# pytorch/audio

Measured on AMD Instinct MI355X. Metric: audio-sec/sec MelSpectrogram (b=256, 16kHz, n_fft=400, n_mels=80), higher is better.
Workload: dtype f32; 1 GPU; MelSpectrogram n_fft=400 hop=160 n_mels=80, batch=256 x 10 s @16 kHz fp32 per GPU (BASELINE configs[1]); per_gpu_batch=256

## Files before the change

### audio_amd/_lib.py

```python
from __future__ import annotations

import ctypes as C
import os
import threading

_HERE = os.path.dirname(os.path.abspath(__file__))
LIB_PATH = os.path.join(_HERE, "lib", "libaudio_amd.so")
if os.environ.get("AAMD_USE_LAB_LIB"):
    LIB_PATH = os.path.join(_HERE, "lib", "libaudio_amd_lab.so")

AAMD_OK = 0
PAD_MODES = {"reflect": 0, "constant": 1, "replicate": 2, "circular": 3}


class StftDesc(C.Structure):
    _fields_ = [
        ("rows", C.c_int64), ("length", C.c_int64), ("row_stride", C.c_int64),
        ("n_fft", C.c_int32), ("hop", C.c_int32), ("pad", C.c_int32), ("center", C.c_int32),
        ("pad_mode", C.c_int32), ("onesided", C.c_int32), ("n_frames", C.c_int32),
        ("scale", C.c_float), ("power", C.c_float),
    ]


class MelBands(C.Structure):
    _fields_ = [
        ("n_mels", C.c_int32), ("max_width", C.c_int32),
        ("lo", C.c_void_p), ("width", C.c_void_p), ("weights", C.c_void_p), ("lane_order", C.c_void_p),
        ("table400", C.c_void_p), ("table_sig", C.c_int32),
    ]


class MfccFused(C.Structure):
    _fields_ = [("dct_frag", C.c_void_p), ("n_mfcc", C.c_int32), ("pass_", C.c_int32), ("multiplier", C.c_float),
                ("amin", C.c_float), ("db_multiplier", C.c_float), ("top_db", C.c_float), ("group_max", C.c_void_p),
                ("rows_per_group", C.c_int64), ("tile_min", C.c_void_p), ("fix_count", C.c_void_p),
                ("tile_list", C.c_void_p)]


class ResampleBands(C.Structure):
    _fields_ = [("n_tiles", C.c_int32), ("tap_span", C.c_int32), ("tap_lo", C.POINTER(C.c_int32))]


_lib = None
# ... 10 lines not shown
class KaldiDesc(C.Structure):
    _fields_ = [("n_samples", C.c_int64), ("n_frames", C.c_int64), ("n_fft", C.c_int32), ("shift", C.c_int32),
                ("win", C.c_int32), ("snip_edges", C.c_int32), ("preemphasis", C.c_float),
                ("remove_dc_offset", C.c_int32), ("raw_energy", C.c_int32), ("energy_floor", C.c_float),
                ("use_power", C.c_int32), ("use_log", C.c_int32), ("energy_col", C.c_int32), ("first_col", C.c_int32),
                ("n_cols", C.c_int32), ("dither", C.c_float), ("noise", C.c_void_p), ("n_utt", C.c_int64),
                ("utt_stride", C.c_int64)]


_SIGS = {
    "aamd_abi_version": (C.c_int, []),
    "aamd_last_error": (C.c_char_p, []),
    "aamd_set_kernel_policy": (C.c_int, [C.c_int]),
    "aamd_mel400_table_dwords": (C.c_int64, [C.c_int32, C.c_int32]),
    "aamd_mel400_table_build": (C.c_int, [C.POINTER(MelBands), _P, _P]),
    "aamd_device_info": (C.c_int, [C.c_char_p, C.c_int32, C.POINTER(C.c_int32), C.POINTER(C.c_int64)]),
    "aamd_box_probe": (C.c_int, [_P, C.c_int32, C.c_int32, _P]),
    "aamd_spectrogram_f32": (C.c_int, [_P, _P, _P, _P, C.POINTER(StftDesc), _P]),
    "aamd_melspectrogram_f32": (C.c_int, [_P, _P, _P, C.POINTER(MelBands), _P, C.POINTER(StftDesc), _P]),
    "aamd_melspectrogram_db_f32": (C.c_int, [_P, _P, _P, C.POINTER(MelBands), _P, C.POINTER(StftDesc), C.c_float,
                                             C.c_float, C.c_float, _P, C.c_int64, _P]),
    "aamd_melspectrogram_lognorm_f32": (C.c_int, [_P, _P, _P, C.POINTER(MelBands), _P, C.POINTER(StftDesc), C.c_float,
                                                  _P, _P, C.c_int64, _P]),
    "aamd_melspectrogram_pcm16_f32": (C.c_int, [_P, _P, _P, C.POINTER(MelBands), _P, C.POINTER(StftDesc), C.c_float,
                                                _P, _P, C.c_int64, _P]),
    "aamd_melspectrogram_pcm16_interleaved_f32": (C.c_int, [_P, C.c_int32, _P, _P, C.POINTER(MelBands), _P,
                                                            C.POINTER(StftDesc), C.c_float, _P, _P, C.c_int64, _P]),
    "aamd_melspectrogram_lowp_f32": (C.c_int, [_P, C.c_int32, _P, _P, C.POINTER(MelBands), _P, C.POINTER(StftDesc), _P]),
    "aamd_spectrogram_grad_f32": (C.c_int, [_P, _P, _P, C.c_int64, C.c_float, _P]),
    "aamd_melspectrogram_grad_f32": (C.c_int, [_P, _P, C.POINTER(MelBands), C.c_int64, C.c_int32, C.c_int32, C.c_float, _P]),
# ... 114 lines not shown
```

### audio_amd/csrc/c_api.hip

```cpp
#include <hip/hip_runtime.h>

#include <atomic>
#include <cmath>
#include <cstdlib>
#include <cstdio>
#include <cstring>
#include <map>
#include <mutex>
#include <utility>
#include <string>

#include "../../include/audio_amd.h"
#include "db_mfcc.h"
#include "f64_paths.h"
#include "feat_post.h"
#include "fftconv.h"
#include "fftconv_os.h"
#include "fftconv_fdr.h"
#include "istft.h"
#include "kaldi_generic.h"
#include "vocoder.h"
#include "stft_pow2.h"
#include "istft400.h"
#include "lfilter.h"
// ... 133 lines not shown
  g.pad_mode = d->pad_mode; g.onesided = d->onesided; g.n_frames = d->n_frames;
  g.n_freq = d->onesided ? d->n_fft / 2 + 1 : d->n_fft;
  g.scale = d->scale; g.power = d->power;
  g.n_stages = plan_radices(d->n_fft, g.radix);
  if (g.n_stages < 0) return fail(AAMD_EUNSUPPORTED, "audio_amd: n_fft has too many prime factors");
  return AAMD_OK;
}

int validate_bands(const aamd_mel_bands* b, int n_freq, MelBandsDev& mb) {
  AAMD_CHECK_ARG(b != nullptr, "null mel bands");
  AAMD_CHECK_ARG(b->n_mels >= 1 && b->max_width >= 1 && b->max_width <= n_freq, "bad mel band table");
  AAMD_CHECK_ARG(b->lo && b->width && b->weights, "null mel band pointers");
  mb.n_mels = b->n_mels; mb.max_width = b->max_width;
  mb.lo = b->lo; mb.width = b->width; mb.weights = b->weights; mb.order = b->lane_order;
  mb.table400 = b->table400;
  mb.table_sig = b->table400 ? b->table_sig : 0;
  return AAMD_OK;
}

template <int EPI, int E>
int launch_pow2(const StftGeom& g, const MelBandsDev& mb, const float* wav, const float* window,
                const float* twiddle, float* out, hipStream_t s) {
  const int64_t pairs_per_row = (g.n_frames + 1) / 2;
  const int64_t n_pairs = g.rows * pairs_per_row;
  if (n_pairs == 0) return AAMD_OK;
  size_t lds = (size_t)p2::kWaves * p2::Cfg<E>::lds_complex * sizeof(p2::C32);
  if (EPI == EPI_MEL && p2::mel_in_lds(mb.n_mels, mb.max_width))
    lds += (size_t)p2::mel_lds_floats(mb.n_mels, mb.max_width) * sizeof(float);
  auto kern = p2::stft_pow2_kernel<E, EPI>;
  if (lds > 48 * 1024)
    AAMD_HIP(hipFuncSetAttribute(reinterpret_cast<const void*>(kern),
// ... 209 lines not shown
  if (n_mels < 1 || max_width < 1) return 0;
  if (m400::mel_ws(max_width) > m400::kMelMaxTaps + 4 || m400::mel_rounds(n_mels) > m400::kMelMaxRounds) return 0;
  return m400::mel_tab_dwords(n_mels, max_width);
}

int aamd_mel400_table_build(const aamd_mel_bands* bands, float* table_out, void* stream) {
  DeviceScope dev_scope_(table_out);
  MelBandsDev mb{};
  int rc = validate_bands(bands, 201, mb);
  if (rc != AAMD_OK) return rc;
  AAMD_CHECK_ARG(table_out != nullptr, "null table buffer");
  if (aamd_mel400_table_dwords(mb.n_mels, mb.max_width) == 0)
    return fail(AAMD_EUNSUPPORTED, "audio_amd: filterbank outside the radix-20x20 kernel (n_mels > 160 or band > 62 bins)");
  mb.table400 = nullptr;
  hipLaunchKernelGGL(m400::mel_tab_build_kernel, dim3(1), dim3(256), 0, (hipStream_t)stream, mb, table_out);
  return launch_check();
}

int aamd_device_info(char* name, int32_t name_len, int32_t* cu_count, int64_t* hbm_bytes) {
  int dev = 0;
  AAMD_HIP(hipGetDevice(&dev));
  hipDeviceProp_t dp;
  AAMD_HIP(hipGetDeviceProperties(&dp, dev));
  if (name && name_len > 0) {
    std::snprintf(name, (size_t)name_len, "%s", dp.gcnArchName);
  }
  if (cu_count) *cu_count = dp.multiProcessorCount;
  if (hbm_bytes) *hbm_bytes = (int64_t)dp.totalGlobalMem;
  return AAMD_OK;
}
// ... 1455 lines not shown
```

### audio_amd/csrc/melspec400.h

```cpp
#pragma once
#include <type_traits>
#include "hd.h"
#include "stft_generic.h"
#include "resample_mfma.h"

namespace aamd {
namespace m400 {

constexpr int kN = 400;
constexpr int kPad = 200;
constexpr int kFramesPerWave = 6;
#ifndef AAMD_M400_WAVES
#define AAMD_M400_WAVES 12
#define AAMD_M400_MINWAVES 3
#endif
constexpr int kWavesPerBlock = AAMD_M400_WAVES;
constexpr int kTOff[20] = {0, 260, 520, 652, 784, 916, 1444, 1576, 128, 388,
                           2104, 2232, 2364, 1708, 1840, 1048, 1180, 1312, 1972, 2492};
constexpr int kTBufDwords = 2492 + 128;
constexpr int kTRow = 44;
constexpr int kTPair = 20 * kTRow;
constexpr int kLdsDwordsPerWave = 3 * kTPair;
constexpr int kPK = 208;
constexpr int kPPair = 416;
// ... 636 lines not shown

template <int NR>
AAMD_HD void mel_regs_load(const LaneConst& c, const MelTab& mt, MelRegs<NR>& h) {
#pragma unroll
  for (int r = 0; r < NR; ++r) {
    const bool on = r < mt.n_rounds;
    const int row = r * kMelSlots + c.pi;
#if defined(__HIP_DEVICE_COMPILE__)
    h.nc[r] = on ? __builtin_amdgcn_readfirstlane(mt.rc[r]) : 0;
#else
    h.nc[r] = on ? mt.rc[r] : 0;
#endif
    const int poff = on ? 2 * mt.lo2[row] : 0;
    const int mel = on ? mt.row_mel[row] : -1;
    h.pm[r] = (int)(((unsigned)mel << 16) | (unsigned)poff);
  }
}

AAMD_HD constexpr int sig_chunks(int sig, int r) { return (sig >> (4 * r)) & 15; }
constexpr int kSigHtk80 = 0x4221, kSigSlaney80 = 0x4211;

template <int NR = kMelMaxRounds, int SIG = 0, bool FENCED = false>
AAMD_HD void phase_c(const LaneConst& c, const MelTab& mt, const float* lds,
                     float (&acc_a)[NR], float (&acc_b)[NR], const MelRegs<NR>* h = nullptr) {
  const float* Pp = lds + kPPair * c.p;
  const float* wt0 = mt.w + c.pi * mt.ws;
#pragma unroll
  for (int r = 0; r < NR; ++r) {
    float sa = 0.0f, sb = 0.0f;
#if defined(__HIP_DEVICE_COMPILE__)
// ... 164 lines not shown
    const float v = mfcc_frag_value(dct, n_mels, n_mfcc, t, s, lane, j);
    const uint16_t hi = rsm::f16_bits(v);
    const uint16_t lo = rsm::f16_bits(v - rsm::f16_value(hi));
    fh[mfcc_frag_piece(t, s, 0, lane) * 8 + j] = hi;
    fh[mfcc_frag_piece(t, s, 1, lane) * 8 + j] = lo;
  }
}

__global__ void __launch_bounds__(256) mel_tab_build_kernel(MelBandsDev mb, float* __restrict__ out) {
  MelTab mt{};
  mel_tab_rounds(threadIdx.x, blockDim.x, mb, out, mt);
  __syncthreads();
  mel_tab_fill(threadIdx.x, blockDim.x, mb, out, mt);
}

template <int LAB, int EPI, int H = 8, typename TIn = float, int NR = kMelMaxRounds, int SIG = 0>
__global__ void __launch_bounds__(64 * kWavesPerBlock, AAMD_M400_MINWAVES)
melspec400_kernel(const TIn* __restrict__ wav, const float* __restrict__ window,
                  const float* __restrict__ tw400, MelBandsDev mb, float* __restrict__ out,
                  int64_t rows, int64_t length, int64_t row_stride, int n_frames, float scale,
                  int tiles_per_row, int64_t n_tiles, int tiles_per_block, int in_aligned,
                  int out_wide, Epi400 epi) {
  extern __shared__ __attribute__((aligned(16))) float smem400[];
  unsigned fix_base = 0, fix_cnt = 0;
#if defined(AAMD_LAB) && defined(AAMD_MFCC_FIXUP_RETURNS)
  if (EPI == EPI400_MFCC && epi.fixup != 0) return;
#endif
  if (EPI == EPI400_MFCC && epi.fixup != 0) {
    int* const cnt = reinterpret_cast<int*>(smem400);
    if (threadIdx.x == 0) *cnt = 0;
// ... 38 lines not shown
#endif
  long long lab_t0 = 0;
  if (LAB & 1024) lab_t0 = wall_clock64();
  if ((LAB & 1048576) && lane == 0) {
    long long* rec = reinterpret_cast<long long*>(epi.fix_count);
    const int w = blockIdx.x * kWavesPerBlock + wave;
    rec[4 * w] = (long long)clock64();
    rec[4 * w + 1] = wall_clock64();
  }
  using HC = Hop<H>;
  constexpr int kHop = HC::hop;
  float* lds = smem400 + wave * HC::lds_dwords;
  const unsigned s_addr = (unsigned)(uintptr_t)(lds + kSOff);

  float* const_tab = smem400 + kWavesPerBlock * HC::lds_dwords;
  const_tab_build(threadIdx.x, blockDim.x, window, tw400, scale, const_tab);
  MelTab mt{};
  const int tab_dwords = (EPI != EPI400_SPEC) ? mel_tab_dwords(mb.n_mels, mb.max_width) : 0;
  int* queue = reinterpret_cast<int*>(const_tab + kConstDwords + tab_dwords);
  constexpr bool kIoWave = (LAB & 16777216) != 0;
  constexpr int kNio = kIoWave ? ((LAB & 67108864) ? 2 : 1) : 0;
  if (threadIdx.x == 0) *queue = kWavesPerBlock - kNio;
  float* frag_lds = const_tab + kConstDwords + tab_dwords + 4;
  constexpr bool kFragLds = (H != 10);
  if (EPI == EPI400_MFCC && (epi.frag_in_lds != 0) != kFragLds) __builtin_trap();
  if (EPI == EPI400_MFCC && kFragLds)
    for (int i = threadIdx.x; i < kMfccFragFloats; i += blockDim.x) frag_lds[i] = epi.dct_frag[i];
  if (EPI != EPI400_SPEC && mb.table400 != nullptr) {
    float* dst = const_tab + kConstDwords;
    for (int i = threadIdx.x; i < tab_dwords; i += blockDim.x) dst[i] = mb.table400[i];
    mel_tab_layout(mb, dst, mt);
    __syncthreads();
  } else {
    if (EPI != EPI400_SPEC) mel_tab_rounds(threadIdx.x, blockDim.x, mb, const_tab + kConstDwords, mt);
    __syncthreads();
    if (EPI != EPI400_SPEC) mel_tab_fill(threadIdx.x, blockDim.x, mb, const_tab + kConstDwords, mt);
    __syncthreads();
  }

  long long lab_t1 = 0;
  if (LAB & 1024) lab_t1 = wall_clock64();
  LaneConst c;
  lane_init(lane, const_tab, c);
  constexpr bool kWinRegs = (EPI != EPI400_MFCC || H != 10) && (((LAB & 8192) != 0) || !(LAB & 262144));
  float winr[20], twr[40];
  if (kWinRegs) {
#pragma unroll
    for (int q = 0; q < 20; ++q) winr[q] = c.win[q];
  }
#ifndef AAMD_M400_TWREG
#define AAMD_M400_TWREG 3
#endif
#ifndef AAMD_M400_TWREG_DB
#define AAMD_M400_TWREG_DB 1
#endif
#ifndef AAMD_M400_TWREG_MFCC
#define AAMD_M400_TWREG_MFCC 2
#endif
  constexpr bool kPlain = H == 8 && std::is_same<TIn, float>::value && LAB == 0;
  constexpr int kTwRegBatches = (LAB & 16384) ? 4
                                : (SIG != 0 && EPI == EPI400_MEL) ? AAMD_M400_TWREG
                                : !kPlain ? 0
                                : EPI == EPI400_SPEC ? 2
                                : (EPI == EPI400_MEL && SIG == 0) ? (NR <= 4 ? 1 : 3)
                                : (EPI == EPI400_MFCC && NR <= 4) ? AAMD_M400_TWREG_MFCC
                                : (EPI == EPI400_MEL_DB && NR <= 4) ? AAMD_M400_TWREG_DB : 0;
  if (kTwRegBatches > 0) {
#pragma unroll
    for (int q = 0; q < 10 * kTwRegBatches; ++q) twr[q] = c.tw[q];
  }
  constexpr bool kHoist = NR <= 4;
  MelRegs<NR> mregs;
  const MelRegs<NR>* mh = nullptr;
  if (EPI != EPI400_SPEC && kHoist) {
    mel_regs_load<NR>(c, mt, mregs);
    mh = &mregs;
  }
  if (SIG != 0) {
    static_assert(SIG == 0 || NR == 4, "filterbank signatures are 4 rounds of 20 mels");
    const int sig_rt = mregs.nc[0] | (mregs.nc[1 % NR] << 4) | (mregs.nc[2 % NR] << 8) | (mregs.nc[3 % NR] << 12);
    if (mt.n_rounds != NR || mt.n_mels != kMelSlots * NR || sig_rt != SIG) __builtin_trap();
  }
  if (EPI == EPI400_MFCC && (mt.n_rounds != NR || mt.n_mels != kMelSlots * NR)) __builtin_trap();
  float nrm_mean[NR], nrm_inv[NR];
  if (EPI == EPI400_MEL_NORM) {
#pragma unroll
    for (int r = 0; r < NR; ++r) {
      const int m = r < mt.n_rounds ? mt.row_mel[r * kMelSlots + c.pi] : -1;
      nrm_mean[r] = m >= 0 ? epi.mean[m] : 0.0f;
      nrm_inv[r] = m >= 0 ? epi.invstd[m] : 0.0f;
    }
  }
  const unsigned long long self_mask = __ballot((c.col == 0) || (c.col == 10));
  using SG = Stage<H, TIn>;
  static_assert(SG::ok, "no staging layout for this hop / input type");
  int spiece[SG::ndma];
#pragma unroll
  for (int k = 0; k < SG::ndma; ++k) spiece[k] = SG::spp * stage_src_piece<H, TIn>(64 * k + lane);

  const int nb = gridDim.x;
  int lb = blockIdx.x;
  if ((nb & 7) == 0) lb = (blockIdx.x & 7) * (nb >> 3) + (blockIdx.x >> 3);
  unsigned blk_first = (unsigned)lb * (unsigned)tiles_per_block;
  unsigned blk_count = 0;
  if (blk_first < (unsigned)n_tiles) {
    blk_count = (unsigned)n_tiles - blk_first;
// ... 155 lines not shown
    for (int i = 0; i < k; ++i) __builtin_amdgcn_s_sleep(17);
  }
  float Xn[HC::nx];
  auto gload = [&](const TileInfo& ti) {
    const TIn* src = wav + (ti.row / InTraits<TIn>::chans) * row_stride + (ti.t0 * kHop - kPad) + (HC::pair_stride * c.p + c.pi);
#pragma unroll
    for (int q = 0; q < HC::nx; ++q) Xn[q] = InTraits<TIn>::get(src + 20 * q, (int)(ti.row % InTraits<TIn>::chans));
  };
  if (LAB & 32768) {
#pragma unroll
    for (int q = 0; q < HC::nx; ++q) Xn[q] = 0.0f;
    if (cur.staged) gload(cur);
  } else if (cur.staged && !(LAB & 8) && !fix) {
    stage_issue(cur);
  }

  long long ph_acc[6] = {0, 0, 0, 0, 0, 0}, ph_t = 0;
  int ph_tiles = 0;
#define AAMD_M400_STAMP(K)                                  \
  if (LAB & 8388608) {                                      \
    const long long now_ = (long long)clock64();            \
    ph_acc[K] += now_ - ph_t;                               \
    ph_t = now_;                                            \
  }
  using mfcc_f32x4 = __attribute__((ext_vector_type(4))) float;
  mfcc_f32x4 cf[kMfccMT];
  const int mfcc_elab = (LAB & 524288) ? epi.lab : 0;
  auto mfcc_finish = [&](int64_t row, int64_t t0) {
#pragma unroll
    for (int t = 0; t < kMfccMT; ++t)
// ... 318 lines not shown
```

### audio_amd/csrc/stft_generic.h

```cpp
#pragma once
#include "hd.h"

namespace aamd {

constexpr int kMaxStages = 16;

struct StftGeom {
  int64_t rows, length, row_stride;
  int n_fft, hop, pad, center, pad_mode, onesided, n_frames, n_freq;
  float scale, power;
  int n_stages;
  int radix[kMaxStages];
};

struct MelBandsDev {
  int n_mels, max_width;
  const int32_t* lo;
  const int32_t* width;
  const float* weights;
  const int32_t* order;
  const float* table400;
  int table_sig;
};

constexpr int kGenThreads = 256;
AAMD_HD int gen_pairs_per_block(int n_fft) {
  int p = 1024 / n_fft;
  return p < 1 ? 1 : (p > 8 ? 8 : p);
}
AAMD_HD int gen_pad(int i) { return i + (i >> 5); }
AAMD_HD int gen_seq_len(int n_fft) { return gen_pad(n_fft - 1) + 1; }
AAMD_HD size_t gen_lds_floats(int n_fft, int n_freq, int pb) {
  return (size_t)2 * n_fft + (size_t)4 * pb * gen_seq_len(n_fft) + (size_t)2 * pb * n_freq;
}
AAMD_HD size_t gen_lds_floats_long(int n_fft, int pb) { return (size_t)4 * pb * gen_seq_len(n_fft); }

template <typename T>
// ... 270 lines not shown
```

### audio_amd/csrc/torch_shim.cpp

```cpp
#include <audio_amd.h>

#include <torch/csrc/inductor/aoti_torch/c/shim.h>
#include <torch/csrc/stable/accelerator.h>
#include <torch/csrc/stable/library.h>
#include <torch/csrc/stable/ops.h>
#include <torch/csrc/stable/tensor.h>
#include <torch/headeronly/core/ScalarType.h>

#include <cmath>
#include <cstdint>
#include <memory>
#include <optional>
#include <string>
#include <type_traits>
#include <vector>

namespace {

using torch::headeronly::ScalarType;
using torch::stable::Tensor;

void check(int rc) {
  STD_TORCH_CHECK(rc == AAMD_OK, aamd_last_error());
}
// ... 60 lines not shown
    b.n_mels = (int32_t)lo.numel();
    b.max_width = (int32_t)weights.size(1);
    b.lo = static_cast<const int32_t*>(lo.data_ptr());
    b.width = static_cast<const int32_t*>(width.data_ptr());
    b.weights = fp(weights);
    b.lane_order = nullptr;
    if (lane_order.has_value()) {
      want_i32(*lane_order, "lane_order");
      same_device(wav, *lane_order);
      b.lane_order = static_cast<const int32_t*>(lane_order->data_ptr());
    }
    b.table400 = nullptr;
    if (table400.has_value()) {
      want_f32(*table400, "table400", 1);
      same_device(wav, *table400);
      STD_TORCH_CHECK(table400->numel() == aamd_mel400_table_dwords(b.n_mels, b.max_width),
                      "audio_amd: table400 does not belong to this band table");
      b.table400 = fp(*table400);
    }
    b.table_sig = b.table400 ? (int32_t)table_sig : 0;
  }
};

Tensor spectrogram(Tensor wav, Tensor window, Tensor twiddle, int64_t n_fft, int64_t hop, int64_t pad, bool center,
                   int64_t pad_mode, bool onesided, int64_t n_frames, double scale, double power) {
  aamd_stft_desc d = make_desc(wav, n_fft, hop, pad, center, pad_mode, onesided, n_frames, scale, power);
  want_f32(window, "window", 1);
  want_f32(twiddle, "twiddle");
  same_device(wav, window);
  same_device(wav, twiddle);
  STD_TORCH_CHECK(window.numel() == n_fft && twiddle.numel() == 2 * n_fft, "audio_amd: window / twiddle size");
  const torch::stable::accelerator::DeviceGuard guard(wav.get_device_index());
  const int64_t n_freq = onesided ? n_fft / 2 + 1 : n_fft;
  Tensor out = torch::stable::new_empty(wav, {d.rows, n_frames, n_freq * (power > 0.0 ? 1 : 2)});
  if (out.numel()) check(aamd_spectrogram_f32(fp(wav), fp(window), fp(twiddle), fpm(out), &d, current_stream(wav)));
// ... 817 lines not shown
```

### audio_amd/functional.py

```python
from __future__ import annotations

import collections
import ctypes as C
import math
import os
import threading
import warnings
import weakref
from typing import List, Optional, Tuple, Union

import numpy as np
import torch
from torch import Tensor

from . import _host
from . import _lib
from . import _shim
from . import _diff
from ._host import create_dct, melscale_fbanks

__all__ = [
    "spectrogram", "inverse_spectrogram", "griffinlim", "phase_vocoder", "pitch_shift", "speed", "amplitude_to_DB", "melscale_fbanks", "create_dct", "resample",
    "lfilter", "biquad", "fftconvolve", "mel_scale", "filtfilt",
    "lowpass_biquad", "highpass_biquad", "allpass_biquad", "bandpass_biquad",
# ... 185 lines not shown
        self.table_sig = 0
        if self.n_freq == 201 and self.lo.is_cuda:
            L = _lib.lib()
            n = L.aamd_mel400_table_dwords(self.n_mels, max_width)
            if n > 0:
                if image is not None and image.shape[0] == n:
                    self.table400 = torch.from_numpy(image).to(device)
                    self.table_sig = _host.mel400_table_signature(image, int(self.n_mels), int(max_width))
                    self.struct.table_sig = self.table_sig
                else:
                    self.table400 = torch.zeros(n, dtype=torch.float32, device=device)
                    with torch.cuda.device(device):
                        _lib.check(L.aamd_mel400_table_build(C.byref(self.struct), self.table400.data_ptr(),
                                                             _lib.current_stream(device)))
                self.struct.table400 = self.table400.data_ptr()


def _mel_bands(fb: Tensor, device) -> MelBandsOnDevice:
    return _tensor_cached(fb, ("bands", str(device)),
                          lambda: MelBandsOnDevice(fb if fb.dtype == torch.float32 else fb.detach().float(), device))


def _get_spec_norms(normalized: Union[str, bool]):
    frame_length_norm, window_norm = False, False
    if isinstance(normalized, str):
        if normalized not in ["frame_length", "window"]:
            raise ValueError("Invalid normalized parameter: {}".format(normalized))
        if normalized == "frame_length":
            frame_length_norm = True
        elif normalized == "window":
# ... 480 lines not shown
                    win_length: int, power: float, normalized, center: bool, pad_mode: str,
                    bands: Optional[MelBandsOnDevice] = None, db=None) -> Tensor:
    _require_device(waveform, "waveform")
    if power is None:
        raise ValueError("audio_amd: MelSpectrogram needs a real power (got None)")
    window = window.to(device=waveform.device, dtype=torch.float32)
    x2 = _rows2d(waveform)
    desc = _stft_desc(x2, pad, window, n_fft, hop_length, power, normalized, center, pad_mode, True)
    if bands is None:
        bands = _mel_bands(fb, waveform.device)
    if bands.n_freq != n_fft // 2 + 1:
        raise RuntimeError(
            f"mat1 and mat2 shapes cannot be multiplied ({desc.n_frames}x{n_fft // 2 + 1} and "
            f"{bands.n_freq}x{bands.n_mels})")
    ops = _ops()
    if ops is not None:
        targs = (x2, _padded_window(window, n_fft), _twiddles(n_fft, waveform.device), bands.lo, bands.width,
                 bands.weights, bands.lane_order, bands.table400, n_fft, hop_length, pad, bool(center), desc.pad_mode, desc.n_frames,
                 desc.scale, desc.power)
        sig = int(bands.table_sig)
        if db is None:
            return ops.mel_spectrogram(*targs, sig)
        multiplier, amin, db_multiplier, group_max, rows_per_group = db
        return ops.mel_spectrogram_db(*targs, multiplier, amin, db_multiplier, group_max, rows_per_group, sig)
    out = torch.empty((desc.rows, desc.n_frames, bands.n_mels), dtype=torch.float32, device=waveform.device)
    if out.numel():
        L = _lib.lib()
        args = (x2.data_ptr(), _padded_window(window, n_fft).data_ptr(), _twiddles(n_fft, waveform.device).data_ptr(),
                C.byref(bands.struct), out.data_ptr(), C.byref(desc))
        if db is None:
            _lib.check(L.aamd_melspectrogram_f32(*args, _lib.current_stream(waveform.device)))
        else:
            multiplier, amin, db_multiplier, group_max, rows_per_group = db
            _lib.check(L.aamd_melspectrogram_db_f32(
                *args, multiplier, amin, db_multiplier, None if group_max is None else group_max.data_ptr(),
                rows_per_group, _lib.current_stream(waveform.device)))
    return out


def _melspectrogram_lowp(waveform: Tensor, pad: int, window: Tensor, fb: Tensor, n_fft: int, hop_length: int,
                         win_length: int, power: float, normalized, center: bool, pad_mode: str) -> Optional[Tensor]:
    if n_fft != 400 or hop_length not in (160, 200) or power != 2.0 or not waveform.is_cuda:
        return None
    dev = waveform.device
# ... 20 lines not shown
def _melspectrogram_plan(waveform: Tensor, pad: int, window: Tensor, fb: Tensor, n_fft: int, hop_length: int,
                         win_length: int, power: float, normalized, center: bool, pad_mode: str):
    ops = _ops()
    if ops is None or power is None:
        return None
    _require_device(waveform, "waveform")
    window_in = window
    window = window.to(device=waveform.device, dtype=torch.float32)
    x2 = _rows2d(waveform)
    if x2.data_ptr() != waveform.data_ptr():
        return None
    desc = _stft_desc(x2, pad, window, n_fft, hop_length, power, normalized, center, pad_mode, True)
    bands = _mel_bands(fb, waveform.device)
    if bands.n_freq != n_fft // 2 + 1:
        return None
    args = (_padded_window(window, n_fft), _twiddles(n_fft, waveform.device), bands.lo, bands.width, bands.weights,
            bands.lane_order, bands.table400, n_fft, hop_length, pad, bool(center), desc.pad_mode, desc.n_frames,
            desc.scale, desc.power, int(bands.table_sig))
    return ops.mel_spectrogram, (x2.shape[0], x2.shape[1]), args, (bands, window, window_in, fb)


def _mel_lognorm(waveform: Tensor, window: Tensor, fb: Tensor, n_fft: int, hop_length: int, gain: float,
                 mean: Tensor, invstddev: Tensor, right_padding: int,
                 bands: Optional[MelBandsOnDevice] = None, interleaved_channels: int = 0) -> Tensor:
    L0 = _lib.lib()
    if interleaved_channels:
        C_ = int(interleaved_channels)
        if waveform.dtype != torch.int16 or waveform.shape[-1] != C_:
            raise ValueError("audio_amd: interleaved PCM must be int16 with a trailing channel dimension")
        n_time = waveform.shape[-2]
        direct = (C_ in (1, 2) and waveform.is_cuda and n_fft == 400 and hop_length in (160, 200) and n_time > 400
                  and not (L0.aamd_set_kernel_policy(-1) & _lib.POLICY_FORCE_GENERIC))
# ... 36 lines not shown
        raise RuntimeError(f"audio_amd: global statistics must have n_mels = {bands.n_mels} entries")
    if pcm16 and not interleaved_channels and not (bands.n_mels <= 160 and bands.max_width <= 62):
        return _mel_lognorm(waveform.to(torch.float32) * (1.0 / 32768.0), window, fb, n_fft, hop_length, gain, mean,
                            invstddev, right_padding, bands)
    T = desc.n_frames
    n_time = x2.shape[-2] if interleaved_channels else x2.shape[1]
    fused_pad = (right_padding > 0 and n_fft == 400 and hop_length in (100, 160, 200) and n_time > 400
                 and bands.n_mels <= 160 and bands.max_width <= 62
                 and not (L0.aamd_set_kernel_policy(-1) & _lib.POLICY_FORCE_GENERIC))
    if interleaved_channels:
        def entry(wav, *rest):
            return L0.aamd_melspectrogram_pcm16_interleaved_f32(wav, int(interleaved_channels), *rest)
    else:
        entry = L0.aamd_melspectrogram_pcm16_f32 if pcm16 else L0.aamd_melspectrogram_lognorm_f32

    def launch(frames: int) -> Tensor:
        out = torch.empty((desc.rows, frames, bands.n_mels), dtype=torch.float32, device=dev)
        if out.numel():
            if frames > T:
                out[:, T:].zero_()
            if T:
                _lib.check(entry(
                    x2.data_ptr(), _padded_window(window, n_fft).data_ptr(), _twiddles(n_fft, dev).data_ptr(),
                    C.byref(bands.struct), out.data_ptr(), C.byref(desc), float(gain), mean.data_ptr(),
                    invstddev.data_ptr(), frames, _lib.current_stream(dev)))
        return out

    if fused_pad:
        try:
            return launch(T + right_padding)
        except RuntimeError as e:
            if "padded feature rows" not in str(e):
                raise
    out = launch(T)
    if right_padding:
        out = torch.nn.functional.pad(out, (0, 0, 0, right_padding))
    return out


# ... 87 lines not shown
            frag = torch.empty((L.aamd_mfcc_frag_floats(),), dtype=torch.float32, device=dev)
            _lib.check(L.aamd_mfcc_frag_build(dct.data_ptr(), bands.n_mels, n_mfcc, frag.data_ptr(), stream))
            state.frag, state.frag_key, state.frag_src = frag, key, weakref.ref(dct)
        n_tiles = int(L.aamd_mfcc_fused_tiles(C.byref(desc)))
        out = torch.empty((desc.rows, desc.n_frames, n_mfcc), dtype=torch.float32, device=dev)
        gmax = _neg_inf.take(n_groups, dev)
        if out.numel() == 0:
            if group_max_hook is not None:
                group_max_hook(gmax)
            return out
        tile_min = torch.empty((n_tiles,), dtype=torch.float32, device=dev)
        count = torch.empty((1,), dtype=torch.int32, device=dev)
        tile_list = torch.empty((n_tiles,), dtype=torch.int32, device=dev)
        f = _lib.MfccFused(state.frag.data_ptr(), n_mfcc, 0, float(db[0]), float(db[1]), float(db[2]), float(top_db),
                           gmax.data_ptr(), max(packed, 1), tile_min.data_ptr(), count.data_ptr(), tile_list.data_ptr())
        args = (x2.data_ptr(), _padded_window(window, n_fft).data_ptr(), _twiddles(n_fft, dev).data_ptr(),
                C.byref(bands.struct), out.data_ptr(), C.byref(desc))
        _lib.check(L.aamd_mfcc_fused_f32(*args, C.byref(f), stream))
        if group_max_hook is not None:
            group_max_hook(gmax)
        f.pass_ = 1
        _lib.check(L.aamd_mfcc_fused_f32(*args, C.byref(f), stream))
        state.last_count, state.last_tiles = count, n_tiles
    return out


def _mfcc(waveform: Tensor, pad: int, window: Tensor, fb: Tensor, dct_mat: Tensor, n_fft: int, hop_length: int,
          win_length: int, power: float, normalized, center: bool, pad_mode: str, log_mels: bool, top_db: float,
          db=(10.0, 1e-10, 0.0), group_max_hook=None, fused_state: Optional[MfccFusedState] = None) -> Tensor:
    lead = tuple(waveform.shape[:-1])
    dev = waveform.device
    if dct_mat.device == dev and dct_mat.dtype == torch.float32 and dct_mat.is_contiguous():
# ... 1557 lines not shown
```

### include/audio_amd.h

```cpp
#ifndef AUDIO_AMD_H
#define AUDIO_AMD_H

#include <stdint.h>

#ifdef __cplusplus
extern "C" {
#endif

#define AAMD_ABI_VERSION 7

enum {
  AAMD_OK = 0,
  AAMD_EINVAL = -1,
  AAMD_EUNSUPPORTED = -2,
  AAMD_EHIP = -3
};

enum { AAMD_PAD_REFLECT = 0, AAMD_PAD_CONSTANT = 1, AAMD_PAD_REPLICATE = 2, AAMD_PAD_CIRCULAR = 3 };

typedef struct aamd_stft_desc {
  int64_t rows;
  int64_t length;
  int64_t row_stride;
  int32_t n_fft;
// ... 4 lines not shown
  int32_t onesided;
  int32_t n_frames;
  float   scale;
  float   power;
} aamd_stft_desc;

typedef struct aamd_mel_bands {
  int32_t n_mels;
  int32_t max_width;
  const int32_t* lo;
  const int32_t* width;
  const float*   weights;
  const int32_t* lane_order;
  const float* table400;
  int32_t table_sig;
} aamd_mel_bands;

int64_t aamd_mel400_table_dwords(int32_t n_mels, int32_t max_width);
int aamd_mel400_table_build(const aamd_mel_bands* bands, float* table_out, void* stream);

enum {
  AAMD_POLICY_FORCE_GENERIC = 1,
  AAMD_POLICY_MEL400_WIDE   = 2,
  AAMD_POLICY_ISTFT_ATOMIC  = 4,
  AAMD_POLICY_RESAMPLE_FP32 = 8,
  AAMD_POLICY_FFTCONV_NO_FDL = 16,
  AAMD_POLICY_FFTCONV_FDL   = 32,
  AAMD_POLICY_FFTCONV_COMPLEX = 64,
  AAMD_POLICY_RESAMPLE_B32 = 128,
  AAMD_POLICY_MEL400_NO_POOL = 256
};
int         aamd_set_kernel_policy(int flags);

int         aamd_abi_version(void);
// ... 211 lines not shown
```

Measured before the change: 37.90 million audio-sec/sec.

## Precompute per-block constant image for n_fft=400 mel kernel prologue

Adds a cached device 'image' holding the window/twiddle constant table, the mel band table, and per-lane register rows (window, twiddles, mel round counts and offsets). It is built once per filterbank/window/scale. The melspec400 kernel then loads lane registers with vector loads and copies the image into LDS with 16-byte copies, instead of rebuilding the constant table and mel registers in every block's prologue. The LDS copy and table checks are deferred until after the first stage issue so they overlap input staging. The cost is extra cached state keyed on window, scale and signature, plus a wider ABI struct.

```diff
diff --git a/audio_amd/_lib.py b/audio_amd/_lib.py
--- a/audio_amd/_lib.py
+++ b/audio_amd/_lib.py
@@ -26,7 +26,7 @@
     _fields_ = [
         ("n_mels", C.c_int32), ("max_width", C.c_int32),
         ("lo", C.c_void_p), ("width", C.c_void_p), ("weights", C.c_void_p), ("lane_order", C.c_void_p),
-        ("table400", C.c_void_p), ("table_sig", C.c_int32),
+        ("table400", C.c_void_p), ("table_sig", C.c_int32), ("image400", C.c_void_p),
     ]
 
 
@@ -67,6 +67,8 @@
     "aamd_set_kernel_policy": (C.c_int, [C.c_int]),
     "aamd_mel400_table_dwords": (C.c_int64, [C.c_int32, C.c_int32]),
     "aamd_mel400_table_build": (C.c_int, [C.POINTER(MelBands), _P, _P]),
+    "aamd_mel400_image_dwords": (C.c_int64, [C.c_int32, C.c_int32]),
+    "aamd_mel400_image_build": (C.c_int, [C.POINTER(MelBands), _P, _P, C.c_float, _P, _P]),
     "aamd_device_info": (C.c_int, [C.c_char_p, C.c_int32, C.POINTER(C.c_int32), C.POINTER(C.c_int64)]),
     "aamd_box_probe": (C.c_int, [_P, C.c_int32, C.c_int32, _P]),
     "aamd_spectrogram_f32": (C.c_int, [_P, _P, _P, _P, C.POINTER(StftDesc), _P]),
diff --git a/audio_amd/csrc/c_api.hip b/audio_amd/csrc/c_api.hip
--- a/audio_amd/csrc/c_api.hip
+++ b/audio_amd/csrc/c_api.hip
@@ -171,7 +171,9 @@
   mb.n_mels = b->n_mels; mb.max_width = b->max_width;
   mb.lo = b->lo; mb.width = b->width; mb.weights = b->weights; mb.order = b->lane_order;
   mb.table400 = b->table400;
-  mb.table_sig = b->table400 ? b->table_sig : 0;
+  mb.image400 = b->image400;
+  mb.table_sig = (b->table400 || b->image400) ? b->table_sig : 0;
+  AAMD_CHECK_ARG(reinterpret_cast<uintptr_t>(b->image400) % 16 == 0, "image400 must be 16-byte aligned");
   return AAMD_OK;
 }
 
@@ -411,6 +413,27 @@
     return fail(AAMD_EUNSUPPORTED, "audio_amd: filterbank outside the radix-20x20 kernel (n_mels > 160 or band > 62 bins)");
   mb.table400 = nullptr;
   hipLaunchKernelGGL(m400::mel_tab_build_kernel, dim3(1), dim3(256), 0, (hipStream_t)stream, mb, table_out);
+  return launch_check();
+}
+
+int64_t aamd_mel400_image_dwords(int32_t n_mels, int32_t max_width) {
+  if (aamd_mel400_table_dwords(n_mels, max_width) == 0) return 0;
+  return m400::image_dwords(n_mels, max_width);
+}
+
+int aamd_mel400_image_build(const aamd_mel_bands* bands, const float* window, const float* twiddle, float scale,
+                            float* image_out, void* stream) {
+  DeviceScope dev_scope_(image_out);
+  MelBandsDev mb{};
+  int rc = validate_bands(bands, 201, mb);
+  if (rc != AAMD_OK) return rc;
+  AAMD_CHECK_ARG(image_out != nullptr && window != nullptr && twiddle != nullptr, "null image, window or twiddle buffer");
+  AAMD_CHECK_ARG(reinterpret_cast<uintptr_t>(image_out) % 16 == 0, "image buffer must be 16-byte aligned");
+  if (aamd_mel400_image_dwords(mb.n_mels, mb.max_width) == 0)
+    return fail(AAMD_EUNSUPPORTED, "audio_amd: filterbank outside the radix-20x20 kernel (n_mels > 160 or band > 62 bins)");
+  mb.image400 = nullptr;
+  hipLaunchKernelGGL(m400::mel_image_build_kernel, dim3(1), dim3(256), 0, (hipStream_t)stream, mb, 1, window, twiddle, scale,
+                     image_out);
   return launch_check();
 }
 
diff --git a/audio_amd/csrc/melspec400.h b/audio_amd/csrc/melspec400.h
--- a/audio_amd/csrc/melspec400.h
+++ b/audio_amd/csrc/melspec400.h
@@ -674,6 +674,27 @@
     const int poff = on ? 2 * mt.lo2[row] : 0;
     const int mel = on ? mt.row_mel[row] : -1;
     h.pm[r] = (int)(((unsigned)mel << 16) | (unsigned)poff);
+  }
+}
+
+constexpr int kLaneRowDwords = 20 + 40 + 4 + 4;
+AAMD_HD int image_tab_dwords(int n_mels, int max_width) { return n_mels > 0 ? mel_tab_dwords(n_mels, max_width) : 0; }
+AAMD_HD int image_lane_off(int n_mels, int max_width) { return (kConstDwords + image_tab_dwords(n_mels, max_width) + 3) & ~3; }
+AAMD_HD int image_dwords(int n_mels, int max_width) { return image_lane_off(n_mels, max_width) + 64 * kLaneRowDwords; }
+AAMD_HD void image_lane_rows(int tid, int nthr, const float* img, bool has_tab, const MelTab& mt, float* rows) {
+  for (int lane = tid; lane < 64; lane += nthr) {
+    LaneConst c;
+    lane_init(lane, img, c);
+    float* r = rows + lane * kLaneRowDwords;
+    for (int q = 0; q < 20; ++q) r[q] = c.win[q];
+    for (int q = 0; q < 40; ++q) r[20 + q] = c.tw[q];
+    int* ri = reinterpret_cast<int*>(r + 60);
+    for (int k = 0; k < 4; ++k) {
+      const bool on = has_tab && k < mt.n_rounds;
+      const int row = k * kMelSlots + c.pi;
+      ri[k] = on ? mt.rc[k] : 0;
+      ri[4 + k] = (int)(((unsigned)(on ? mt.row_mel[row] : -1) << 16) | (unsigned)(on ? 2 * mt.lo2[row] : 0));
+    }
   }
 }
 
@@ -868,6 +889,28 @@
   mel_tab_fill(threadIdx.x, blockDim.x, mb, out, mt);
 }
 
+__global__ void __launch_bounds__(256) mel_image_build_kernel(MelBandsDev mb, int has_bands, const float* __restrict__ window,
+                                                              const float* __restrict__ tw400, float scale,
+                                                              float* __restrict__ out) {
+  const_tab_build(threadIdx.x, blockDim.x, window, tw400, scale, out);
+  float* tab = out + kConstDwords;
+  MelTab mt{};
+  if (has_bands) {
+    if (mb.table400 != nullptr) {
+      const int n = mel_tab_dwords(mb.n_mels, mb.max_width);
+      for (int i = threadIdx.x; i < n; i += blockDim.x) tab[i] = mb.table400[i];
+      mel_tab_layout(mb, tab, mt);
+    } else {
+      mel_tab_rounds(threadIdx.x, blockDim.x, mb, tab, mt);
+      __syncthreads();
+      mel_tab_fill(threadIdx.x, blockDim.x, mb, tab, mt);
+    }
+  }
+  __syncthreads();
+  image_lane_rows(threadIdx.x, blockDim.x, out, has_bands != 0, mt,
+                  out + image_lane_off(has_bands ? mb.n_mels : 0, mb.max_width));
+}
+
 template <int LAB, int EPI, int H = 8, typename TIn = float, int NR = kMelMaxRounds, int SIG = 0>
 __global__ void __launch_bounds__(64 * kWavesPerBlock, AAMD_M400_MINWAVES)
 melspec400_kernel(const TIn* __restrict__ wav, const float* __restrict__ window,
@@ -936,7 +979,10 @@
   const unsigned s_addr = (unsigned)(uintptr_t)(lds + kSOff);
 
   float* const_tab = smem400 + kWavesPerBlock * HC::lds_dwords;
-  const_tab_build(threadIdx.x, blockDim.x, window, tw400, scale, const_tab);
+  constexpr bool kImgHead = !AAMD_M400_POOLS && (LAB & ~1024) == 0;
+  static_assert((kWavesPerBlock * HC::lds_dwords) % 4 == 0, "the constant tables start on a 16-byte boundary in LDS");
+  const bool img = kImgHead && mb.image400 != nullptr;
+  if (!img) const_tab_build(threadIdx.x, blockDim.x, window, tw400, scale, const_tab);
   MelTab mt{};
   const int tab_dwords = (EPI != EPI400_SPEC) ? mel_tab_dwords(mb.n_mels, mb.max_width) : 0;
   int* queue = reinterpret_cast<int*>(const_tab + kConstDwords + tab_dwords);
@@ -946,9 +992,14 @@
   float* frag_lds = const_tab + kConstDwords + tab_dwords + 4;
   constexpr bool kFragLds = (H != 10);
   if (EPI == EPI400_MFCC && (epi.frag_in_lds != 0) != kFragLds) __builtin_trap();
-  if (EPI == EPI400_MFCC && kFragLds)
-    for (int i = threadIdx.x; i < kMfccFragFloats; i += blockDim.x) frag_lds[i] = epi.dct_frag[i];
-  if (EPI != EPI400_SPEC && mb.table400 != nullptr) {
+  auto frag_copy = [&]() {
+    if (EPI == EPI400_MFCC && kFragLds)
+      for (int i = threadIdx.x; i < kMfccFragFloats; i += blockDim.x) frag_lds[i] = epi.dct_frag[i];
+  };
+  if (!img) frag_copy();
+  if (img) {
+    if (EPI != EPI400_SPEC) mel_tab_layout(mb, const_tab + kConstDwords, mt);
+  } else if (EPI != EPI400_SPEC && mb.table400 != nullptr) {
     float* dst = const_tab + kConstDwords;
     for (int i = threadIdx.x; i < tab_dwords; i += blockDim.x) dst[i] = mb.table400[i];
     mel_tab_layout(mb, dst, mt);
@@ -966,9 +1017,19 @@
   lane_init(lane, const_tab, c);
   constexpr bool kWinRegs = (EPI != EPI400_MFCC || H != 10) && (((LAB & 8192) != 0) || !(LAB & 262144));
   float winr[20], twr[40];
+  const float* lrow = img ? mb.image400 + image_lane_off(EPI != EPI400_SPEC ? mb.n_mels : 0, mb.max_width) + lane * kLaneRowDwords
+                          : nullptr;
   if (kWinRegs) {
-#pragma unroll
-    for (int q = 0; q < 20; ++q) winr[q] = c.win[q];
+    if (img) {
+#pragma unroll
+      for (int q = 0; q < 20; q += 4) {
+        const F4 v = *reinterpret_cast<const F4*>(lrow + q);
+        winr[q] = v.x; winr[q + 1] = v.y; winr[q + 2] = v.z; winr[q + 3] = v.w;
+      }
+    } else {
+#pragma unroll
+      for (int q = 0; q < 20; ++q) winr[q] = c.win[q];
+    }
   }
 #ifndef AAMD_M400_TWREG
 #define AAMD_M400_TWREG 3
@@ -988,23 +1049,48 @@
                                 : (EPI == EPI400_MFCC && NR <= 4) ? AAMD_M400_TWREG_MFCC
                                 : (EPI == EPI400_MEL_DB && NR <= 4) ? AAMD_M400_TWREG_DB : 0;
   if (kTwRegBatches > 0) {
-#pragma unroll
-    for (int q = 0; q < 10 * kTwRegBatches; ++q) twr[q] = c.tw[q];
+    if (img) {
+#pragma unroll
+      for (int q = 0; q + 4 <= 10 * kTwRegBatches; q += 4) {
+        const F4 v = *reinterpret_cast<const F4*>(lrow + 20 + q);
+        twr[q] = v.x; twr[q + 1] = v.y; twr[q + 2] = v.z; twr[q + 3] = v.w;
+      }
+      if ((10 * kTwRegBatches) & 2) {
+        constexpr int q = (10 * kTwRegBatches) & ~3;
+        const F2 v = *reinterpret_cast<const F2*>(lrow + 20 + q);
+        twr[q] = v.x; twr[q + 1] = v.y;
+      }
+    } else {
+#pragma unroll
+      for (int q = 0; q < 10 * kTwRegBatches; ++q) twr[q] = c.tw[q];
+    }
   }
   constexpr bool kHoist = NR <= 4;
   MelRegs<NR> mregs;
   const MelRegs<NR>* mh = nullptr;
+  int img_nc[4] = {0, 0, 0, 0};
   if (EPI != EPI400_SPEC && kHoist) {
-    mel_regs_load<NR>(c, mt, mregs);
+    if (img) {
+      const int4 a = *reinterpret_cast<const int4*>(lrow + 60), b = *reinterpret_cast<const int4*>(lrow + 64);
+      img_nc[0] = a.x; img_nc[1] = a.y; img_nc[2] = a.z; img_nc[3] = a.w;
+      const int pmv[4] = {b.x, b.y, b.z, b.w};
+#pragma unroll
+      for (int r = 0; r < NR; ++r) mregs.pm[r] = pmv[r & 3];
+    } else {
+      mel_regs_load<NR>(c, mt, mregs);
+    }
     mh = &mregs;
   }
+  auto table_checks = [&]() {
   if (SIG != 0) {
     static_assert(SIG == 0 || NR == 4, "filterbank signatures are 4 rounds of 20 mels");
     const int sig_rt = mregs.nc[0] | (mregs.nc[1 % NR] << 4) | (mregs.nc[2 % NR] << 8) | (mregs.nc[3 % NR] << 12);
     if (mt.n_rounds != NR || mt.n_mels != kMelSlots * NR || sig_rt != SIG) __builtin_trap();
   }
   if (EPI == EPI400_MFCC && (mt.n_rounds != NR || mt.n_mels != kMelSlots * NR)) __builtin_trap();
+  };
   float nrm_mean[NR], nrm_inv[NR];
+  auto norm_load = [&]() {
   if (EPI == EPI400_MEL_NORM) {
 #pragma unroll
     for (int r = 0; r < NR; ++r) {
@@ -1012,6 +1098,11 @@
       nrm_mean[r] = m >= 0 ? epi.mean[m] : 0.0f;
       nrm_inv[r] = m >= 0 ? epi.invstd[m] : 0.0f;
     }
+  }
+  };
+  if (!img) {
+    table_checks();
+    norm_load();
   }
   const unsigned long long self_mask = __ballot((c.col == 0) || (c.col == 10));
   using SG = Stage<H, TIn>;
@@ -1197,6 +1288,21 @@
   } else if (cur.staged && !(LAB & 8) && !fix) {
     stage_issue(cur);
   }
+  if (img) {
+    const int n4 = (kConstDwords + (EPI != EPI400_SPEC ? mel_tab_dwords(mb.n_mels, mb.max_width) : 0)) >> 2;
+    const F4* src = reinterpret_cast<const F4*>(mb.image400);
+    F4* dst = reinterpret_cast<F4*>(const_tab);
+    for (int i = threadIdx.x; i < n4; i += blockDim.x) dst[i] = src[i];
+    frag_copy();
+    stage_wait();
+    __syncthreads();
+    if (EPI != EPI400_SPEC && kHoist) {
+#pragma unroll
+      for (int r = 0; r < NR; ++r) mregs.nc[r] = __builtin_amdgcn_readfirstlane(img_nc[r & 3]);
+    }
+    table_checks();
+    norm_load();
+  }
 
   long long ph_acc[6] = {0, 0, 0, 0, 0, 0}, ph_t = 0;
   int ph_tiles = 0;
diff --git a/audio_amd/csrc/stft_generic.h b/audio_amd/csrc/stft_generic.h
--- a/audio_amd/csrc/stft_generic.h
+++ b/audio_amd/csrc/stft_generic.h
@@ -21,6 +21,7 @@
   const int32_t* order;
   const float* table400;
   int table_sig;
+  const float* image400;
 };
 
 constexpr int kGenThreads = 256;
diff --git a/audio_amd/csrc/torch_shim.cpp b/audio_amd/csrc/torch_shim.cpp
--- a/audio_amd/csrc/torch_shim.cpp
+++ b/audio_amd/csrc/torch_shim.cpp
@@ -98,11 +98,15 @@
     if (table400.has_value()) {
       want_f32(*table400, "table400", 1);
       same_device(wav, *table400);
-      STD_TORCH_CHECK(table400->numel() == aamd_mel400_table_dwords(b.n_mels, b.max_width),
-                      "audio_amd: table400 does not belong to this band table");
-      b.table400 = fp(*table400);
+      const int64_t n_tab = aamd_mel400_table_dwords(b.n_mels, b.max_width);
+      if (n_tab > 0 && table400->numel() == aamd_mel400_image_dwords(b.n_mels, b.max_width)) {
+        b.image400 = fp(*table400);
+      } else {
+        STD_TORCH_CHECK(table400->numel() == n_tab, "audio_amd: table400 does not belong to this band table");
+        b.table400 = fp(*table400);
+      }
     }
-    b.table_sig = b.table400 ? (int32_t)table_sig : 0;
+    b.table_sig = (b.table400 || b.image400) ? (int32_t)table_sig : 0;
   }
 };
 
diff --git a/audio_amd/functional.py b/audio_amd/functional.py
--- a/audio_amd/functional.py
+++ b/audio_amd/functional.py
@@ -223,6 +223,25 @@
                         _lib.check(L.aamd_mel400_table_build(C.byref(self.struct), self.table400.data_ptr(),
                                                              _lib.current_stream(device)))
                 self.struct.table400 = self.table400.data_ptr()
+
+    def image_for(self, window400: Tensor, twiddle: Tensor, scale: float):
+        if self.table400 is None or window400.numel() != 400:
+            return self.table400, self.struct
+
+        def make():
+            L = _lib.lib()
+            dev = self.table400.device
+            image = torch.empty(L.aamd_mel400_image_dwords(int(self.n_mels), int(self.max_width)), dtype=torch.float32,
+                                device=dev)
+            with torch.cuda.device(dev):
+                _lib.check(L.aamd_mel400_image_build(C.byref(self.struct), window400.data_ptr(), twiddle.data_ptr(),
+                                                     float(scale), image.data_ptr(), _lib.current_stream(dev)))
+            st = _lib.MelBands(self.struct.n_mels, self.struct.max_width, self.struct.lo, self.struct.width,
+                               self.struct.weights, self.struct.lane_order, self.struct.table400, self.struct.table_sig,
+                               image.data_ptr())
+            return image, st, self
+
+        return _tensor_cached(window400, ("m400img", id(self), float(scale), int(self.struct.table_sig)), make)[:2]
 
 
 def _mel_bands(fb: Tensor, device) -> MelBandsOnDevice:
@@ -733,9 +752,12 @@
             f"mat1 and mat2 shapes cannot be multiplied ({desc.n_frames}x{n_fft // 2 + 1} and "
             f"{bands.n_freq}x{bands.n_mels})")
     ops = _ops()
+    image, bstruct = bands.table400, bands.struct
+    if n_fft == 400:
+        image, bstruct = bands.image_for(_padded_window(window, n_fft), _twiddles(n_fft, waveform.device), desc.scale)
     if ops is not None:
         targs = (x2, _padded_window(window, n_fft), _twiddles(n_fft, waveform.device), bands.lo, bands.width,
-                 bands.weights, bands.lane_order, bands.table400, n_fft, hop_length, pad, bool(center), desc.pad_mode, desc.n_frames,
+                 bands.weights, bands.lane_order, image, n_fft, hop_length, pad, bool(center), desc.pad_mode, desc.n_frames,
                  desc.scale, desc.power)
         sig = int(bands.table_sig)
         if db is None:
@@ -746,7 +768,7 @@
     if out.numel():
         L = _lib.lib()
         args = (x2.data_ptr(), _padded_window(window, n_fft).data_ptr(), _twiddles(n_fft, waveform.device).data_ptr(),
-                C.byref(bands.struct), out.data_ptr(), C.byref(desc))
+                C.byref(bstruct), out.data_ptr(), C.byref(desc))
         if db is None:
             _lib.check(L.aamd_melspectrogram_f32(*args, _lib.current_stream(waveform.device)))
         else:
@@ -797,8 +819,11 @@
     bands = _mel_bands(fb, waveform.device)
     if bands.n_freq != n_fft // 2 + 1:
         return None
+    image = bands.table400
+    if n_fft == 400:
+        image = bands.image_for(_padded_window(window, n_fft), _twiddles(n_fft, waveform.device), desc.scale)[0]
     args = (_padded_window(window, n_fft), _twiddles(n_fft, waveform.device), bands.lo, bands.width, bands.weights,
-            bands.lane_order, bands.table400, n_fft, hop_length, pad, bool(center), desc.pad_mode, desc.n_frames,
+            bands.lane_order, image, n_fft, hop_length, pad, bool(center), desc.pad_mode, desc.n_frames,
             desc.scale, desc.power, int(bands.table_sig))
     return ops.mel_spectrogram, (x2.shape[0], x2.shape[1]), args, (bands, window, window_in, fb)
 
@@ -865,6 +890,10 @@
     else:
         entry = L0.aamd_melspectrogram_pcm16_f32 if pcm16 else L0.aamd_melspectrogram_lognorm_f32
 
+    bstruct = bands.struct
+    if n_fft == 400:
+        bstruct = bands.image_for(_padded_window(window, n_fft), _twiddles(n_fft, dev), desc.scale)[1]
+
     def launch(frames: int) -> Tensor:
         out = torch.empty((desc.rows, frames, bands.n_mels), dtype=torch.float32, device=dev)
         if out.numel():
@@ -873,7 +902,7 @@
             if T:
                 _lib.check(entry(
                     x2.data_ptr(), _padded_window(window, n_fft).data_ptr(), _twiddles(n_fft, dev).data_ptr(),
-                    C.byref(bands.struct), out.data_ptr(), C.byref(desc), float(gain), mean.data_ptr(),
+                    C.byref(bstruct), out.data_ptr(), C.byref(desc), float(gain), mean.data_ptr(),
                     invstddev.data_ptr(), frames, _lib.current_stream(dev)))
         return out
 
@@ -991,8 +1020,9 @@
         tile_list = torch.empty((n_tiles,), dtype=torch.int32, device=dev)
         f = _lib.MfccFused(state.frag.data_ptr(), n_mfcc, 0, float(db[0]), float(db[1]), float(db[2]), float(top_db),
                            gmax.data_ptr(), max(packed, 1), tile_min.data_ptr(), count.data_ptr(), tile_list.data_ptr())
+        bstruct = bands.image_for(_padded_window(window, n_fft), _twiddles(n_fft, dev), desc.scale)[1]
         args = (x2.data_ptr(), _padded_window(window, n_fft).data_ptr(), _twiddles(n_fft, dev).data_ptr(),
-                C.byref(bands.struct), out.data_ptr(), C.byref(desc))
+                C.byref(bstruct), out.data_ptr(), C.byref(desc))
         _lib.check(L.aamd_mfcc_fused_f32(*args, C.byref(f), stream))
         if group_max_hook is not None:
             group_max_hook(gmax)
diff --git a/include/audio_amd.h b/include/audio_amd.h
--- a/include/audio_amd.h
+++ b/include/audio_amd.h
@@ -42,10 +42,14 @@
   const int32_t* lane_order;
   const float* table400;
   int32_t table_sig;
+  const float* image400;
 } aamd_mel_bands;
 
 int64_t aamd_mel400_table_dwords(int32_t n_mels, int32_t max_width);
 int aamd_mel400_table_build(const aamd_mel_bands* bands, float* table_out, void* stream);
+int64_t aamd_mel400_image_dwords(int32_t n_mels, int32_t max_width);
+int aamd_mel400_image_build(const aamd_mel_bands* bands, const float* window, const float* twiddle, float scale,
+                            float* image_out, void* stream);
 
 enum {
   AAMD_POLICY_FORCE_GENERIC = 1,
```

After: 35.12 million audio-sec/sec. -7.3%, worse.
